# alenzhao/Mitty

Measured on NVIDIA B200. Metric: read pairs/sec (2x150, FASTQ-formatted, corrupted), higher is better.
Workload: dtype u8

## Files before the change

mitty_b200/csrc/mg_api.cu:

```cuda
#include <algorithm>
#include <cmath>
#include <cstdarg>
#include <cstdio>
#include <cstring>
#include <ctime>
#include <cstdlib>
#include <condition_variable>
#include <deque>
#include <map>
#include <memory>
#include <mutex>
#include <string>
#include <thread>
#include <vector>

#include "../../include/mitty_b200.h"
#include "mg_internal.h"

namespace {

struct DevBuf {
  void *p = nullptr;
  size_t cap = 0;
  ~DevBuf() { if (p) cudaFree(p); }
// ... 43 lines not shown
  uint32_t *d_eblk = nullptr;
  int n_blk = 0; int64_t hap_words = 0, hap_len = 0;
  std::vector<MgSegOut> segs;
  std::vector<int64_t> seg_start1;
  mg_ctx *owner = nullptr;
  ~Copy();
};

struct Batch {
  std::unique_ptr<Region> R;
  std::unique_ptr<Copy> C;
};

const int BLK_SHIFT = 8;

}

struct mg_ctx {
  int device = 0;
  cudaStream_t stream = nullptr;
  bool own_stream = false;
  std::string err;
  DevBuf m_tlen, m_bq, m_phred, m_alias[2], m_tlen_alias;
  bool has_tlen_alias = false;
  int n_tlen = 0, n_mates = 0, n_cycles = 0, n_bq = 0, rlen = 0;
  std::vector<uint32_t> h_alias[2]; int a_kshift[2] = {0, 0}, a_code9[2] = {0, 0}, a_rows[2] = {0, 0};
  std::vector<std::pair<void *, size_t>> pool;
  size_t pool_bytes = 0;
  std::map<void *, size_t> block_size;
  std::map<int64_t, std::unique_ptr<Region>> regions;
  std::map<int64_t, std::unique_ptr<Copy>> copies;
  std::map<int64_t, std::unique_ptr<Batch>> batches;
  int64_t next_id = 1;
  DevBuf s_raw, s_exc, s_ts, s_u, s_fo, s_tsorted, s_partial, s_state, s_out[2][2], s_str, s_plan, s_sample[3];
  DevBuf c_in[2], c_out[2], c_nl[2], c_cnt, c_sz[2], c_off[2], c_tmp, c_draw[4];
  DevBuf b_units, b_arr;
  HostBuf h_stage;
  cudaEvent_t ev0 = nullptr, ev1 = nullptr, ev2 = nullptr;
  cudaStream_t copy_stream = nullptr;
  cudaEvent_t ev_d2h[2] = {nullptr, nullptr};
  int ob = 0;
  int last_ob = 0; int64_t last_bytes = 0;
  double plan_ms = 0;
  double emit_ms = 0; int64_t emit_launches = 0, emit_bytes = 0, total_launches = 0;
  struct DrainJob {
    mg_sink *sink; int producer; int64_t unit; int ob; int64_t bytes;
    std::shared_ptr<std::vector<int64_t>> units, base;
  };
  std::thread drain_thread;
  std::mutex dmu; std::condition_variable dcv;
  std::deque<DrainJob> djobs;
  int dbusy[2] = {0, 0};
  bool dstop = false, dfailed = false;
  std::string derr;
  cudaEvent_t ev_drain[2] = {nullptr, nullptr};
  double d_wait_slot_ms = 0, d_wait_copy_ms = 0, d_idle_ms = 0; int64_t d_bytes = 0;
};

namespace {

int fail(mg_ctx *c, int code, const char *fmt, ...) {
  char buf[512];
  va_list ap; va_start(ap, fmt); vsnprintf(buf, sizeof buf, fmt, ap); va_end(ap);
  if (c) c->err = buf;
  return code;
}

// ... 629 lines not shown
  MgUnitParams P; const Copy *C;
  int rc = fill_unit_params(ctx, d, P, &C, false);
  if (rc) return rc;
  if (!d->qname_prefix || !d->qname_mid) return fail(ctx, MG_EINVAL, "qname_prefix / qname_mid missing");
  if (d->corrupt && d->mode != MG_MODE_PHILOX) return fail(ctx, MG_EINVAL, "fused corruption draws from Philox: use mg_corrupt_fastq for deterministic mode");
  if (d->corrupt && ctx->rlen > ctx->n_cycles) return fail(ctx, MG_EINDEX, "read length %d exceeds the model's %d cycles", ctx->rlen, ctx->n_cycles);
  if (d->corrupt && ctx->n_mates < 2) return fail(ctx, MG_EINVAL, "paired corruption needs a 2-mate model");
  const size_t n = (size_t)d->n_candidates;
  const int pl = (int)strlen(d->qname_prefix), ml = (int)strlen(d->qname_mid);
  const int L = ctx->rlen;

  if (pl > MG_QN_MAX || ml > MG_QN_MAX) return fail(ctx, MG_EVALUE, "sample / chromosome name too long for the qname buffers (%d)", MG_QN_MAX);
  mg_qn_const(P.qn, reinterpret_cast<const uint8_t *>(d->qname_prefix), pl, reinterpret_cast<const uint8_t *>(d->qname_mid), ml, L);
  P.qn_len = pl + ml;
  {
    static const bool lsu = getenv("MG_COPYOUT_LSU") != nullptr;
    P.bulk = lsu ? 0 : 1;
  }
  P.corrupt = d->corrupt;
  P.cor.kshift = ctx->a_kshift[0]; P.cor.code9 = ctx->a_code9[0];
  P.cor.alias = ctx->m_alias[0].as<uint32_t>();
  P.cor.n_cycles = ctx->n_cycles; P.cor.n_mates = ctx->n_mates;
  P.cor.k0 = d->corrupt_seed; P.cor.k1 = d->unit_seed ^ 0x636f7231u;
  P.L_nd = mg_ndigits32((uint32_t)L);

  P.n_tiles = (int)((n + MG_PLAN_TILE - 1) / MG_PLAN_TILE);
  int stage = 32 * (2 * L + 5 + 96);
  if (stage > 48 * 1024) stage = 48 * 1024;
  P.stage_cap = stage & ~15;
  int smem = 0;
  const int grid = mg_unit_grid(L, d->corrupt ? 1 + P.cor.code9 : 0, P.stage_cap, &smem);
  if (grid <= 0) return fail(ctx, MG_EVALUE, "the emit kernel's staging area (%d bytes for reads of %d bases) exceeds the shared memory of this device", smem, L);

  const size_t state_bytes = 48 + 16 * (size_t)std::max(P.n_tiles, 1);
  CU(ctx->s_state.need(state_bytes));
  uint8_t *sb = ctx->s_state.as<uint8_t>();
  P.totals = reinterpret_cast<unsigned long long *>(sb);
  P.tile_counter = reinterpret_cast<uint32_t *>(sb + 32);
  P.descA = reinterpret_cast<unsigned long long *>(sb + 48);
  P.descB = P.descA + std::max(P.n_tiles, 1);
  CU(ctx->s_plan.need(sizeof(MgPlan) * std::max<size_t>(n, 1)));
  P.plan = ctx->s_plan.as<MgPlan>();

  size_t est = n * (size_t)(2 * L + 5 + pl + ml + 12 + 2 * 36) / 6 * 5 + 4096;
  const bool want_out = (out1 != nullptr) || (out2 != nullptr);
  unsigned long long tot[4] = {0, 0, 0, 0};
  CU(cudaMemsetAsync(sb, 0, state_bytes, ctx->stream));
  CU(cudaEventRecord(ctx->ev2, ctx->stream));
  mg_launch_plan(P, ctx->stream);
  CU(cudaGetLastError());
  {
    std::unique_lock<std::mutex> lk(ctx->dmu);
    while (ctx->dbusy[ctx->ob] > 0 && !ctx->dfailed) ctx->dcv.wait(lk);
    if (ctx->dfailed) return fail(ctx, MG_EVALUE, "output sink: %s", ctx->derr.c_str());
  }
  for (int attempt = 0; attempt < 2; attempt++) {
    DevBuf *ob = ctx->s_out[ctx->ob];
    if (ob[0].cap < est || ob[1].cap < est) CU(cudaStreamSynchronize(ctx->copy_stream));
    CU(ob[0].need(est)); CU(ob[1].need(est));
    P.out[0] = ob[0].as<uint8_t>(); P.out[1] = ob[1].as<uint8_t>();
    P.cap = std::min(ob[0].cap, ob[1].cap);
    CU(cudaStreamWaitEvent(ctx->stream, ctx->ev_d2h[ctx->ob], 0));
    CU(cudaEventRecord(ctx->ev0, ctx->stream));
    mg_launch_unit(P, grid, smem, ctx->stream);
    CU(cudaEventRecord(ctx->ev1, ctx->stream));
    CU(cudaGetLastError());
    CU(cudaMemcpyAsync(tot, P.totals, sizeof tot, cudaMemcpyDeviceToHost, ctx->stream));
    CU(cudaStreamSynchronize(ctx->stream));
    if (P.n_tiles) {
      float ms = 0, ms_plan = 0;
      cudaEventElapsedTime(&ms, ctx->ev0, ctx->ev1);
      if (attempt == 0) { cudaEventElapsedTime(&ms_plan, ctx->ev2, ctx->ev0); ctx->plan_ms += ms_plan; ctx->total_launches++; }
      ctx->emit_ms += ms; ctx->emit_launches++; ctx->total_launches++;
      ctx->emit_bytes += 2 * (int64_t)tot[2];
    }
    if (!tot[3]) break;
    if (attempt == 1) return fail(ctx, MG_ECUDA, "internal: output overflow after regrow");
    est = (size_t)tot[2] + 4096;
    CU(cudaMemsetAsync(P.totals + 3, 0, 8, ctx->stream));
  }
  ctx->last_ob = ctx->ob; ctx->last_bytes = (int64_t)tot[2];
  if (n_bytes) *n_bytes = (int64_t)tot[2];
  if (n_templates) *n_templates = (int64_t)tot[1];
  if (n_te_kept) *n_te_kept = (int64_t)tot[0];
  if (!want_out) ctx->ob ^= 1;
  if (want_out) {
    if ((int64_t)tot[2] > cap) return fail(ctx, MG_ECAP, "output needs %lld bytes per file, caller gave %lld", (long long)tot[2], (long long)cap);
    if (out1 && tot[2]) CU(cudaMemcpyAsync(out1, P.out[0], (size_t)tot[2], cudaMemcpyDeviceToHost, ctx->copy_stream));
    if (out2 && tot[2]) CU(cudaMemcpyAsync(out2, P.out[1], (size_t)tot[2], cudaMemcpyDeviceToHost, ctx->copy_stream));
    CU(cudaEventRecord(ctx->ev_d2h[ctx->ob], ctx->copy_stream));
    ctx->ob ^= 1;
    if (wait_copies) CU(cudaStreamSynchronize(ctx->copy_stream));
  }
  return MG_OK;
}

int mg_unit_generate(mg_ctx *ctx, const mg_unit_desc *d, uint8_t *out1, uint8_t *out2, int64_t cap, int64_t *n_bytes,
                     int64_t *n_templates, int64_t *n_te_kept) {
  return unit_generate(ctx, d, out1, out2, cap, n_bytes, n_templates, n_te_kept, true);
}

int mg_unit_generate_async(mg_ctx *ctx, const mg_unit_desc *d, uint8_t *out1, uint8_t *out2, int64_t cap, int64_t *n_bytes,
                           int64_t *n_templates, int64_t *n_te_kept) {
  return unit_generate(ctx, d, out1, out2, cap, n_bytes, n_templates, n_te_kept, false);
}
// ... 488 lines not shown
```

mitty_b200/csrc/mg_core.cuh:

```cuda
#pragma once
#include <stdint.h>

#if defined(__CUDACC__)
#define MG_HD __host__ __device__ __forceinline__
#else
#define MG_HD inline
#endif
#if defined(__CUDACC__)
#define MG_NI static __host__ __device__ __noinline__ __attribute__((unused))
#else
#define MG_NI static __attribute__((noinline, unused))
#endif
#if defined(__CUDA_ARCH__)
#define MG_UNROLL _Pragma("unroll")
#define MG_NOUNROLL _Pragma("unroll 1")
#else
#define MG_UNROLL
#define MG_NOUNROLL
#endif


struct alignas(16) MgNode {
  uint32_t key;
  int32_t pr;
// ... 338 lines not shown
  MgTok A, B;
  mg_tok_num(v, pre, npre, A, B);
  w.append(A); w.append(B);
}

template <class SP>
MG_HD void mg_put_small(MgStream<SP> &w, uint32_t v, uint32_t pre, uint32_t npre) {
  if (v >= 10000u) { mg_put_num(w, v, pre, npre); return; }
  const uint32_t d = mg_dec4(v), x = d ^ 0x30303030u;
  uint32_t lz;
#if defined(__CUDA_ARCH__)
  lz = (x & 0x00FFFFFFu) ? ((uint32_t)__ffs((int)x) - 1u) >> 3 : 3u;
#else
  lz = (x & 0x00FFFFFFu) ? ((uint32_t)__builtin_ctz(x)) >> 3 : 3u;
#endif
  const uint32_t dig = d >> (8u * lz), ps = 8u * npre;
  MgTok t;
  t.lo = pre | (dig << ps); t.hi = mg_funnel_l(dig, 0u, ps); t.n = npre + 4u - lz;
  w.append(t);
}

MG_HD MgTok mg_tok(uint32_t lo, uint32_t hi, uint32_t n) { MgTok t; t.lo = lo; t.hi = hi; t.n = n; return t; }

template <class W>
MG_HD void mg_put_u32(W &w, uint32_t v) {
  uint64_t acc = 0;
  int n = 0;
  do { uint32_t q = v / 10u; acc = (acc << 4) | (v - q * 10u); v = q; n++; } while (v);
  for (; n; n--) { w.put((uint8_t)('0' + ((uint32_t)acc & 15u))); acc >>= 4; }
}


template <class NP, class BP>
MG_NI int mg_find_node(NP nodes, BP blk, int blk_shift, int n_blk, int n_nodes, uint32_t x) {
  uint32_t b = x >> blk_shift;
  if ((int)b >= n_blk) b = (uint32_t)(n_blk - 1);
  int lo = (int)blk[b];
  int hi = ((int)b + 1 < n_blk) ? (int)blk[b + 1] : n_nodes - 1;
  while (lo < hi) {
    int mid = (lo + hi + 1) >> 1;
    if (nodes[mid].key <= x) lo = mid; else hi = mid - 1;
  }
  return lo;
}

template <class NP>
MG_HD int mg_last_node(NP nodes, int n0, int n_nodes, uint32_t x, int L) {
  const uint32_t last = x + (uint32_t)L - 1u;
  int n1 = n0;
  while (n1 + 1 < n_nodes && nodes[n1 + 1].key <= last) n1++;
  return n1;
}

MG_HD int32_t mg_read_pos(const MgNode &f, bool single, uint32_t x) {
  if (f.op == 'I') return single ? f.pr - 1 : f.pr;
  const int64_t ps0 = (int64_t)f.key - (f.op == 'D' ? 1 : 0);
  return (int32_t)((int64_t)x - ps0 + (int64_t)f.pr);
}

MG_HD int32_t mg_cigar_len(const MgNode &n, uint32_t x, int L) {
  if (n.op == 'D') return n.oplen;
  int64_t a = (int64_t)x - (int64_t)n.key; if (a < 0) a = 0;
  int64_t b = (int64_t)x + L - (int64_t)n.key; if ((int64_t)n.oplen < b) b = n.oplen;
  return (int32_t)(b - a);
}

template <class W>
MG_HD void mg_put_i32(W &w, int32_t v) {
  if (v < 0) { w.put('-'); mg_put_u32(w, (uint32_t)(-(int64_t)v)); } else mg_put_u32(w, (uint32_t)v);
}

MG_HD int mg_nchars_i32(int32_t v) {
  const bool neg = v < 0;
  return (neg ? 1 : 0) + mg_ndigits32(neg ? (uint32_t)(-(int64_t)v) : (uint32_t)v);
}

template <class NP>
MG_NI uint32_t mg_read_fields_len(NP nodes, int n0, int n1, uint32_t x, int L, int L_nd) {
  const MgNode f = nodes[n0];
  const bool single = (n0 == n1);
  uint32_t n = 2u + 1u + (uint32_t)mg_nchars_i32(mg_read_pos(f, single, x)) + 1u + (uint32_t)L_nd + 1u + 1u;
  if (single && f.op == '=') return n + (uint32_t)L_nd + 1u;
  if (single && f.op == 'I')
    return n + 1u + (uint32_t)mg_nchars_i32((int32_t)((int64_t)x - (int64_t)f.key)) + 1u + (uint32_t)L_nd + 1u + (uint32_t)mg_nchars_i32(f.oplen);
  uint32_t nv = 0;
  for (int k = n0; k <= n1; k++) {
    const MgNode nd = nodes[k];
    n += (uint32_t)mg_nchars_i32(mg_cigar_len(nd, x, L)) + 1u;
    if (nd.op != '=') {
      n += (nv ? 1u : 0u) + (nd.op == 'X' ? 1u : nd.op == 'I' ? (uint32_t)mg_nchars_i32(nd.oplen) : (uint32_t)mg_nchars_i32(-nd.oplen));
      nv++;
    }
  }
  return n;
}

template <class W, class NP>
MG_HD void mg_fmt_read(W &w, NP nodes, int n0, int n1, uint32_t x, int L, int strand) {
  const MgNode f = nodes[n0];
  const bool single = (n0 == n1);
  w.put('|'); w.put((uint8_t)('0' + strand));
  w.put('|'); mg_put_i32(w, mg_read_pos(f, single, x));
  w.put('|'); mg_put_u32(w, (uint32_t)L);
  w.put('|');
  if (single && f.op == '=') {
    mg_put_u32(w, (uint32_t)L); w.put('='); w.put('|');
    return;
  }
  if (single && f.op == 'I') {
    w.put('>'); mg_put_i32(w, (int32_t)((int64_t)x - (int64_t)f.key)); w.put(':'); mg_put_u32(w, (uint32_t)L); w.put('I');
  } else {
    for (int k = n0; k <= n1; k++) {
      const MgNode n = nodes[k];
      mg_put_i32(w, mg_cigar_len(n, x, L)); w.put((uint8_t)n.op);
    }
  }
  w.put('|');
  bool first = true;
  for (int k = n0; k <= n1; k++) {
    const MgNode n = nodes[k];
    if (n.op == '=') continue;
    if (!first) w.put(',');
    first = false;
    if (n.op == 'X') w.put('0');
    else mg_put_i32(w, n.op == 'I' ? n.oplen : -n.oplen);
  }
}
// ... 146 lines not shown

template <class EP>
MG_HD int mg_exc_first(EP exc, int n_exc, uint32_t x) {
  int lo = 0, hi = n_exc;
  while (lo < hi) {
    int mid = (lo + hi) >> 1;
    if ((uint64_t)exc[mid].start + exc[mid].len <= (uint64_t)x) lo = mid + 1; else hi = mid;
  }
  return lo;
}

struct MgExcView {
  const MgExc *p; const uint32_t *blk; int shift, n_blk;
  MG_HD const MgExc &operator[](int k) const { return p[k]; }
};

MG_HD int mg_exc_first(MgExcView exc, int n_exc, uint32_t x) {
  int lo = 0, hi = n_exc;
  if (exc.blk) {
    uint32_t b = x >> exc.shift;
    if ((int)b > exc.n_blk - 1) b = (uint32_t)(exc.n_blk - 1);
    lo = (int)exc.blk[b]; hi = (int)exc.blk[b + 1];
    if (hi > n_exc) hi = n_exc;
    if (lo > hi) lo = hi;
  }
  while (lo < hi) {
    int mid = (lo + hi) >> 1;
    if ((uint64_t)exc.p[mid].start + exc.p[mid].len <= (uint64_t)x) lo = mid + 1; else hi = mid;
  }
  return lo;
}

template <class EP>
MG_NI int mg_count_N(EP exc, int n_exc, uint32_t x, int L, bool &touch) {
  int cnt = 0;
  touch = false;
  for (int k = mg_exc_first(exc, n_exc, x); k < n_exc; k++) {
    MgExc e = exc[k];
    if ((uint64_t)e.start >= (uint64_t)x + L) break;
    touch = true;
    if (e.byte != 'N') continue;
    uint64_t a = e.start > x ? e.start : x;
    uint64_t b = (uint64_t)e.start + e.len < (uint64_t)x + L ? (uint64_t)e.start + e.len : (uint64_t)x + L;
    cnt += (int)(b - a);
  }
  return cnt;
}

template <class HP>
MG_HD uint8_t mg_exc_byte(const MgExc &e, HP hap, uint64_t i) {
  if (e.byte != MG_EXC_CASE) return (uint8_t)e.byte;
  return (uint8_t)("acgt"[(hap[i >> 4] >> (2 * (i & 15))) & 3u]);
}

template <class HP>
struct MgCodeCursor {
  HP hap; uint64_t wi; uint32_t wv;
  MG_HD explicit MgCodeCursor(HP h) : hap(h), wi(~0ull), wv(0u) {}
  MG_HD uint32_t at(uint64_t i) {
    if ((i >> 4) != wi) { wi = i >> 4; wv = hap[wi]; }
    return (wv >> (2u * ((uint32_t)i & 15u))) & 3u;
  }
};

#define MG_CASE_WORDS 6
struct MgCaseMask {
  uint32_t m[MG_CASE_WORDS];
  MG_HD void clear() { MG_UNROLL for (int w = 0; w < MG_CASE_WORDS; w++) m[w] = 0u; }
  MG_HD void set(uint32_t lo, uint32_t hi) {
    MG_UNROLL
    for (int w = 0; w < MG_CASE_WORDS; w++) {
      const uint32_t l = lo > 32u * w ? lo - 32u * w : 0u, h = hi < 32u * w + 32u ? (hi > 32u * w ? hi - 32u * w : 0u) : 32u;
      if (l < h) m[w] |= (h - l == 32u ? 0xFFFFFFFFu : ((1u << (h - l)) - 1u) << l);
    }
  }
  MG_HD uint32_t next4() {
    const uint32_t b = m[0] & 15u;
    MG_UNROLL
    for (int w = 0; w + 1 < MG_CASE_WORDS; w++) m[w] = mg_funnel_r(m[w], m[w + 1], 4u);
// ... 348 lines not shown
```

mitty_b200/csrc/mg_internal.h:

```cpp
#pragma once
#include <cuda_runtime.h>
#include <stdint.h>
#include "mg_core.cuh"

#define MG_PLAN_TILE 256
#define MG_CTA 128
#define MG_TLEN_K 1024
#define MG_QN_MAX 192
#define MG_HAP_PAD 8

enum { MG_MODE_PHILOX = 0, MG_MODE_DET = 1, MG_MODE_EXPLICIT = 2 };

struct alignas(16) MgPlan {
  uint32_t xa, xb;
  int32_t n0a, n0b;
  uint32_t dn;
  uint32_t fo_sz;
  uint64_t off;
};

#define MG_BATCH_MAXC 2048
struct MgBatchUnit {
  MgTok pre[4], mid[4];
  int n_pre, n_mid;
  uint32_t qn_len;
  uint32_t seed;
  uint32_t x0, hap_len;
  uint32_t n_cand, plan_off;
  int64_t draw_off;
  int64_t p_min;
};

struct MgUnitParams {
  const uint32_t *hap;
  uint32_t hap_len;
  int64_t p_min;
  const MgNode *nodes; int n_nodes;
  const uint32_t *blk; int blk_shift; int n_blk;
  const MgExc *exc; int n_exc;
  const uint32_t *eblk;
  const double *cum_tlen; int n_tlen; int rlen;
  const uint32_t *tlen_alias;
  int mode; uint32_t n_cand;
  const int64_t *ts_in;
  const double *u_tlen;
  const int64_t *tl_in;
  const int8_t *fo_in;
  const uint32_t *ts_sorted;
  uint32_t key_tlen0, key_tlen1, key_perm0, key_perm1, perm_bits;
  MgQnConst qn;
  int qn_len;
  int bulk;
  uint8_t *out[2]; uint64_t cap;
  MgPlan *plan;
  int corrupt; MgCorruptCtx cor;
  int L_nd;
  unsigned long long *descA, *descB; uint32_t *tile_counter;
  unsigned long long *totals;
  int n_tiles; int stage_cap;
  const MgBatchUnit *bunits; int n_bunits;
  const long long *kept_base, *byte_base;
  long long *unit_kept, *unit_bytes, *unit_te;
  double inv_log1mp;
};

struct MgUnitKeys { uint32_t gap0, gap1, tlen0, tlen1, perm0, perm1, perm_bits; };
__host__ __device__ inline MgUnitKeys mg_unit_keys(uint32_t seed, uint32_t n_cand) {
  MgUnitKeys k;
  k.gap0 = seed; k.gap1 = 0x67617031u;
  k.tlen0 = seed; k.tlen1 = 0x746c6531u;
  k.perm0 = seed ^ 0x7368756bu; k.perm1 = seed * 0x9E3779B1u + 0x66656973u;
  k.perm_bits = mg_perm_bits(n_cand);
  return k;
}

struct MgSampleParams {
  MgUnitParams u;
  int64_t *ts_out; int64_t *te_out; int8_t *fo_out;
};

struct MgCorruptParams {
  const uint8_t *in[2]; uint8_t *out[2];
  const int64_t *nl[2];
  const int64_t *out_off[2];
  int64_t n_rec; int n_files;
  int64_t first;
  const double *cum_bq; int n_cycles, n_bq; const double *phred;
  int mode;
  MgCorruptCtx cor;
  const double *bq_rnd, *call_rnd; const uint8_t *base_rnd; const int64_t *draw_off;
// ... 15 lines not shown
  int32_t ends_in_d;
  uint32_t node0, n_nodes;
  uint32_t pad;
};
struct MgWalkSummary {
  unsigned long long err;
  long long n_nodes, hap_len;
  int32_t ends_in_d, bad;
};

struct MgWalkParams {
  const int64_t *pos, *oplen, *alt_off; const uint8_t *op;
  int n_var;
  const MgSeg *segs; int n_seg; MgSegOut *seg_out;
  uint32_t *nxt, *jump[2]; uint8_t *mark; int32_t *pred;
  int64_t *packed, *scanned, *scan_tmp;
  MgNode *nodes; uint32_t *node_alt;
  MgWalkSummary *sum;
};

int mg_launch_walk(const MgWalkParams &W, cudaStream_t st);
void mg_launch_exc_count(const MgNode *nodes, const uint32_t *node_alt, const MgWalkSummary *sum, int max_nodes,
                         const uint8_t *alt_pool, const MgExc *rexc, int n_rexc, int64_t *cnt, cudaStream_t st);
void mg_launch_exc_write(const MgNode *nodes, const uint32_t *node_alt, const MgWalkSummary *sum, int max_nodes,
                         const uint8_t *alt_pool, const MgExc *rexc, int n_rexc, int64_t *off, MgExc *out, cudaStream_t st);
void mg_launch_hap_build(const uint32_t *ref, const uint8_t *alt_pool, const MgNode *nodes, const uint32_t *node_alt,
                         int n_nodes, const uint32_t *blk, int blk_shift, int n_blk, uint32_t hap_len, uint32_t *hap, int64_t hap_words,
                         cudaStream_t st);
void mg_launch_blk_table(const MgNode *nodes, int n_nodes, uint32_t *blk, int n_blk, int blk_shift, cudaStream_t st);
void mg_launch_eblk_table(const MgExc *exc, int n_exc, uint32_t *eblk, int n_entries, int blk_shift, cudaStream_t st);
void mg_launch_gap_scan(uint32_t n, double p, uint32_t k0, uint32_t k1, uint32_t *ts_sorted, unsigned long long *partial,
                        cudaStream_t st);
int mg_unit_grid(int L, int corrupt, int stage_cap, int *smem_bytes);
void mg_launch_plan(const MgUnitParams &P, cudaStream_t st);
void mg_launch_unit(const MgUnitParams &P, int grid, int smem_bytes, cudaStream_t st);
void mg_launch_batch_plan(const MgUnitParams &P, cudaStream_t st);
int mg_batch_grid(int L, int corrupt, int stage_cap, int *smem_bytes);
void mg_launch_batch_emit(const MgUnitParams &P, int grid, int smem_bytes, cudaStream_t st);
void mg_launch_sample(const MgSampleParams &P, cudaStream_t st);
void mg_launch_scan_i64(const int64_t *in, int64_t *out, int64_t n, int64_t *tmp, cudaStream_t st);
int64_t mg_scan_tmp_elems(int64_t n);
void mg_launch_nl_count(const uint8_t *buf, int64_t len, int64_t *cnt, cudaStream_t st);
void mg_launch_nl_write(const uint8_t *buf, int64_t len, const int64_t *off, int64_t *nl, cudaStream_t st);
int64_t mg_nl_chunks(int64_t len);
void mg_launch_corrupt_sizes(const MgCorruptParams &P, int64_t *sz0, int64_t *sz1, cudaStream_t st);
void mg_launch_corrupt(const MgCorruptParams &P, cudaStream_t st);
void mg_launch_corrupt_staged(const MgCorruptParams &P, bool bulk, cudaStream_t st);
int mg_corrupt_stage_cap(void);
```

mitty_b200/csrc/mg_kernels.cu:

```cuda
#include <algorithm>
#include <cstdlib>
#include "mg_internal.h"

#define FULL 0xffffffffu


__device__ __forceinline__ uint32_t warp_incl_scan_u32(uint32_t v, int lane) {
#pragma unroll
  for (int d = 1; d < 32; d <<= 1) {
    uint32_t n = __shfl_up_sync(FULL, v, d);
    if (lane >= d) v += n;
  }
  return v;
}

__device__ __forceinline__ unsigned long long warp_sum_u64(unsigned long long v) {
#pragma unroll
  for (int d = 16; d >= 1; d >>= 1) v += __shfl_xor_sync(FULL, v, d);
  return v;
}

__device__ __forceinline__ unsigned long long ld_vol64(const unsigned long long *p) {
  return *(const volatile unsigned long long *)p;
}
__device__ __forceinline__ void st_vol64(unsigned long long *p, unsigned long long v) {
  *(volatile unsigned long long *)p = v;
}


__global__ void __launch_bounds__(256) k_pack_ref(const uint8_t *__restrict__ raw, int64_t len, uint32_t *__restrict__ packed,
                                                  uint32_t *exc_cnt, int64_t *exc_start, uint8_t *exc_byte,
                                                  int64_t *exc_end, uint32_t exc_cap) {
  int64_t w = (int64_t)blockIdx.x * blockDim.x + threadIdx.x;
  int64_t base = w * 16;
  if (base >= len) return;
  uint8_t c[18];
  c[0] = base > 0 ? raw[base - 1] : 0;
  if (base + 16 <= len) {
    uint4 v = *reinterpret_cast<const uint4 *>(raw + base);
    uint32_t q[4] = {v.x, v.y, v.z, v.w};
#pragma unroll
    for (int i = 0; i < 16; i++) c[1 + i] = (uint8_t)(q[i >> 2] >> (8 * (i & 3)));
  } else {
#pragma unroll
    for (int i = 0; i < 16; i++) c[1 + i] = (base + i < len) ? raw[base + i] : (uint8_t)'A';
  }
  c[17] = (base + 16 < len) ? raw[base + 16] : 0;
  uint32_t word = 0;
#pragma unroll
  for (int i = 0; i < 16; i++) {
    int64_t pos = base + i;
    if (pos >= len) break;
    uint32_t code = mg_base_code(c[1 + i]);
    if (code > 3) {
      const uint32_t lc = mg_base_code((uint8_t)(c[1 + i] ^ 0x20));
      const bool soft = c[1 + i] >= 'a' && lc <= 3;
      bool is_start, is_end;
      if (soft) {
        const bool prev_soft = pos > 0 && c[i] >= 'a' && mg_base_code((uint8_t)(c[i] ^ 0x20)) <= 3;
        const bool next_soft = pos < len - 1 && c[2 + i] >= 'a' && mg_base_code((uint8_t)(c[2 + i] ^ 0x20)) <= 3;
// ... 467 lines not shown
    }
    c.fo = r.v[2] & 1u;
  } else {
    c.ts_rel = P.ts_in[j] - P.p_min;
    tl = (P.mode == MG_MODE_DET) ? (int64_t)mg_lower_bound_f64(P.cum_tlen, P.n_tlen, P.u_tlen[j]) : P.tl_in[j];
  }
  if (tl < P.rlen) tl = P.rlen;
  c.te_rel = c.ts_rel + tl;
  c.k1 = (c.te_rel < (int64_t)P.hap_len) && (c.ts_rel >= 0);
  return c;
}

__global__ void __launch_bounds__(256) k_sample(MgSampleParams S) {
  __shared__ uint32_t s_tlen[MG_TLEN_K];
  if (S.u.mode == MG_MODE_PHILOX && S.u.tlen_alias)
    for (int i = threadIdx.x; i < MG_TLEN_K; i += blockDim.x) s_tlen[i] = S.u.tlen_alias[i];
  __syncthreads();
  for (uint32_t j = blockIdx.x * blockDim.x + threadIdx.x; j < S.u.n_cand; j += gridDim.x * blockDim.x) {
    Cand c = sample_candidate(S.u, s_tlen, j);
    S.ts_out[j] = c.ts_rel + S.u.p_min;
    S.te_out[j] = c.k1 ? c.te_rel + S.u.p_min : -1;
    S.fo_out[j] = (int8_t)c.fo;
  }
}

void mg_launch_sample(const MgSampleParams &P, cudaStream_t st) {
  if (P.u.n_cand == 0) return;
  int grid = (int)((P.u.n_cand + 255) / 256);
  if (grid > 148 * 8) grid = 148 * 8;
  k_sample<<<grid, 256, 0, st>>>(P);
}


struct Agg { unsigned long long c1, c2, by; };

#define DESC_FLAG(x) ((uint32_t)((x) >> 62))
#define DESC_MASK62 ((1ull << 62) - 1ull)

#define LOOKBACK_WIN 128
__device__ Agg tile_lookback(const MgUnitParams &P, int tile, int lane) {
  constexpr int Q = LOOKBACK_WIN / 32;
  Agg ex = {0, 0, 0};
  int idx = tile - 1;
  while (true) {
    unsigned long long a[Q], b[Q];
#pragma unroll
    for (int q = 0; q < Q; q++) {
      const int t = idx - 32 * q - lane;
      a[q] = 2ull << 62; b[q] = 2ull << 62;
      if (t >= 0) { a[q] = ld_vol64(P.descA + t); b[q] = ld_vol64(P.descB + t); }
    }
#pragma unroll
    for (int q = 0; q < Q; q++) {
      const int t = idx - 32 * q - lane;
      while (t >= 0 && (DESC_FLAG(a[q]) == 0 || DESC_FLAG(a[q]) != DESC_FLAG(b[q]))) {
        a[q] = ld_vol64(P.descA + t); b[q] = ld_vol64(P.descB + t);
      }
    }
    __syncwarp();
    int stop = LOOKBACK_WIN;
#pragma unroll
    for (int q = Q - 1; q >= 0; q--) {
      const uint32_t pm = __ballot_sync(FULL, DESC_FLAG(a[q]) == 2);
      if (pm) stop = 32 * q + __ffs(pm) - 1;
    }
    unsigned long long c1 = 0, c2 = 0, by = 0;
#pragma unroll
    for (int q = 0; q < Q; q++) {
      if (32 * q + lane <= stop) {
        c1 += (a[q] >> 31) & 0x7FFFFFFFull; c2 += a[q] & 0x7FFFFFFFull; by += b[q] & DESC_MASK62;
      }
    }
    ex.c1 += warp_sum_u64(c1); ex.c2 += warp_sum_u64(c2); ex.by += warp_sum_u64(by);
    if (stop < LOOKBACK_WIN) break;
    idx -= LOOKBACK_WIN;
  }
  return ex;
}

#define PLAN_THREADS 256

__global__ void __launch_bounds__(PLAN_THREADS, 6) k_unit_plan(const __grid_constant__ MgUnitParams P) {
  __shared__ uint32_t s_tlen[MG_TLEN_K];
  __shared__ uint4 s_hold[2][PLAN_THREADS];
  __shared__ uint2 s_hold2[2][PLAN_THREADS], s_ex[PLAN_THREADS];
  __shared__ uint32_t s_wc[2][PLAN_THREADS / 32], s_ws[2][PLAN_THREADS / 32];
  __shared__ unsigned long long s_base[2][3];
  __shared__ uint32_t s_tile[2];
  const int t = threadIdx.x, lane = t & 31, wid = t >> 5;
  const int L = P.rlen;
  if (P.mode == MG_MODE_PHILOX && P.tlen_alias) {
#pragma unroll 1
    for (int i = t; i < MG_TLEN_K; i += PLAN_THREADS) s_tlen[i] = P.tlen_alias[i];
  }
  if (t == 0) s_tile[0] = atomicAdd(P.tile_counter, 1u);
  __syncthreads();
  int tile = (int)s_tile[0], prev = -1;
  uint32_t prev_c1 = 0, prev_c2 = 0, prev_sz = 0;
#pragma unroll 1
  for (int k = 0;; k++) {
    const int cur = k & 1;
    const bool live = tile < P.n_tiles;
    if (t == 0 && live) s_tile[cur ^ 1] = atomicAdd(P.tile_counter, 1u);
    const uint32_t j = (uint32_t)tile * PLAN_THREADS + t;
    bool k1 = false, k2 = false, ta = false, tb = false;
    uint32_t xa = 0, xb = 0, fo = 0, sz = 0;
    int n0a = 0, n1a = 0, n0b = 0, n1b = 0;
    if (live && j < P.n_cand) {
      Cand c = sample_candidate(P, s_tlen, j);
      k1 = c.k1; fo = c.fo;
      if (k1) {
        xa = (uint32_t)c.ts_rel; xb = (uint32_t)(c.te_rel - L);
        k2 = true;
        if (P.n_exc) {
          const MgExcView ev = {P.exc, P.eblk, P.blk_shift, P.n_blk};
          const int na = mg_count_N(ev, P.n_exc, xa, L, ta), nb = mg_count_N(ev, P.n_exc, xb, L, tb);
          k2 = na <= 2 && nb <= 2;
        }
        if (k2) {
          n0a = mg_find_node(P.nodes, P.blk, P.blk_shift, P.n_blk, P.n_nodes, xa);
          n1a = mg_last_node(P.nodes, n0a, P.n_nodes, xa, L);
          n0b = mg_find_node(P.nodes, P.blk, P.blk_shift, P.n_blk, P.n_nodes, xb);
          n1b = mg_last_node(P.nodes, n0b, P.n_nodes, xb, L);
          sz = (uint32_t)P.qn_len + mg_read_fields_len(P.nodes, n0a, n1a, xa, L, P.L_nd) +
               mg_read_fields_len(P.nodes, n0b, n1b, xb, L, P.L_nd) + 2u * (uint32_t)L + 5u;
        }
      }
    }
    s_hold[cur][t] = make_uint4(xa, xb, (uint32_t)n0a, (uint32_t)n0b);
    s_hold2[cur][t] = make_uint2((uint32_t)(n1a - n0a) | ((uint32_t)(n1b - n0b) << 16),
                                 (fo << 31) | ((ta ? 1u : 0u) << 30) | ((tb ? 1u : 0u) << 29) | sz);
    const uint32_t cpk = (k1 ? 1u : 0u) | (k2 ? 0x10000u : 0u);
    const uint32_t ic = warp_incl_scan_u32(cpk, lane), is = warp_incl_scan_u32(sz, lane);
    if (lane == 31) { s_wc[cur][wid] = ic; s_ws[cur][wid] = is; }
    if (wid == 0 && prev >= 0) {
      Agg ex = {0, 0, 0};
      if (prev > 0) ex = tile_lookback(P, prev, lane);
      if (lane == 0) {
        const unsigned long long i1 = ex.c1 + prev_c1, i2 = ex.c2 + prev_c2, ib = ex.by + prev_sz;
        if (prev > 0) {
          st_vol64(P.descA + prev, (2ull << 62) | (i1 << 31) | i2);
          st_vol64(P.descB + prev, (2ull << 62) | ib);
        }
        s_base[cur ^ 1][0] = ex.c1; s_base[cur ^ 1][1] = ex.c2; s_base[cur ^ 1][2] = ex.by;
        if (prev == P.n_tiles - 1) { P.totals[0] = i1; P.totals[1] = i2; P.totals[2] = ib + mg_digit_sum(i2); }
      }
    }
    __syncthreads();
    if (prev >= 0) {
      const uint2 h1 = s_hold2[cur ^ 1][t];
      if (h1.y & 0x1FFFFFFFu) {
        const uint4 h0 = s_hold[cur ^ 1][t];
        const uint2 ex = s_ex[t];
        const unsigned long long base1 = s_base[cur ^ 1][0], base2 = s_base[cur ^ 1][1];
        const unsigned long long rank = base2 + (ex.x >> 16);
        const unsigned long long off = s_base[cur ^ 1][2] + ex.y + mg_digit_sum(rank);
        const uint32_t my_fo = (P.mode == MG_MODE_PHILOX) ? h1.y >> 31 : (uint32_t)(P.fo_in[base1 + (ex.x & 0xFFFFu)] & 1);
        MgPlan pl;
        pl.xa = h0.x; pl.xb = h0.y; pl.n0a = (int32_t)h0.z; pl.n0b = (int32_t)h0.w;
        pl.dn = h1.x;
        pl.fo_sz = (my_fo << 31) | ((h1.y & 0x7FFFFFFFu) + (uint32_t)mg_ndigits32((uint32_t)(rank + 1)));
        pl.off = off;
        P.plan[rank] = pl;
      }
    }
    if (!live) break;
    uint32_t oc = 0, os = 0, tc = 0, ts_ = 0;
#pragma unroll
    for (int w = 0; w < PLAN_THREADS / 32; w++) {
      if (w < wid) { oc += s_wc[cur][w]; os += s_ws[cur][w]; }
      tc += s_wc[cur][w]; ts_ += s_ws[cur][w];
    }
    const uint32_t ec = oc + ic - cpk, es = os + is - sz;
    prev_c1 = tc & 0xFFFFu; prev_c2 = tc >> 16; prev_sz = ts_;
    if (t == 0) {
      const unsigned long long fl = tile == 0 ? 2ull << 62 : 1ull << 62;
      st_vol64(P.descA + tile, fl | ((unsigned long long)prev_c1 << 31) | prev_c2);
      st_vol64(P.descB + tile, fl | prev_sz);
    }
    s_ex[t] = make_uint2(ec, es);
    prev = tile;
    tile = (int)s_tile[cur ^ 1];
  }
}

void mg_launch_plan(const MgUnitParams &P, cudaStream_t st) {
  if (P.n_tiles == 0) return;
  static const int resident = [] {
    int dev = 0, sms = 0, per_sm = 0;
    cudaGetDevice(&dev);
    cudaDeviceGetAttribute(&sms, cudaDevAttrMultiProcessorCount, dev);
    cudaOccupancyMaxActiveBlocksPerMultiprocessor(&per_sm, k_unit_plan, PLAN_THREADS, 0);
    return std::max(1, sms * per_sm);
  }();
  k_unit_plan<<<std::min(P.n_tiles, resident), PLAN_THREADS, 0, st>>>(P);
}

__global__ void __launch_bounds__(PLAN_THREADS) k_batch_plan(const __grid_constant__ MgUnitParams P) {
  __shared__ uint32_t s_ts[MG_BATCH_MAXC];
  __shared__ uint32_t s_tlen[MG_TLEN_K];
  __shared__ unsigned long long s_w64[PLAN_THREADS / 32];
  __shared__ uint32_t s_wc[PLAN_THREADS / 32], s_ws[PLAN_THREADS / 32];
  __shared__ unsigned long long s_carry[3];
  const int t = threadIdx.x, lane = t & 31, wid = t >> 5;
  const int L = P.rlen;
  const MgBatchUnit U = P.bunits[blockIdx.x];
  const uint32_t n = U.n_cand;
  const MgUnitKeys K = mg_unit_keys(U.seed, n);
  if (P.mode == MG_MODE_PHILOX) {
    if (P.tlen_alias) for (int i = t; i < MG_TLEN_K; i += PLAN_THREADS) s_tlen[i] = P.tlen_alias[i];
    uint32_t g[8];
    unsigned long long sum = 0;
    const uint32_t i0 = (uint32_t)t * 8u;
    if (i0 < n) { gaps8(i0, n, P.inv_log1mp, K.gap0, K.gap1, g); for (int q = 0; q < 8; q++) sum += g[q]; }
    else { for (int q = 0; q < 8; q++) g[q] = 0; }
    unsigned long long x = sum;
#pragma unroll
    for (int d = 1; d < 32; d <<= 1) { unsigned long long y = __shfl_up_sync(FULL, x, d); if (lane >= d) x += y; }
    if (lane == 31) s_w64[wid] = x;
    __syncthreads();
    unsigned long long run = x - sum;
    for (int w = 0; w < wid; w++) run += s_w64[w];
    for (int q = 0; q < 8; q++) {
      run += g[q];
      if (i0 + q < n) { const unsigned long long v = run + 1; s_ts[i0 + q] = v > 0xFFFFFFFFull ? 0xFFFFFFFFu : (uint32_t)v; }
    }
  }
  if (t == 0) { s_carry[0] = 0; s_carry[1] = 0; s_carry[2] = 0; }
  __syncthreads();
  for (uint32_t c0 = 0; c0 < n; c0 += PLAN_THREADS) {
// ... 720 lines not shown
```

Baseline: 1.419 billion.

## Replace single-pass decoupled-lookback plan kernel with count/scan/place three-kernel pipeline

Replaces the persistent plan kernel, which used dynamic tile counters and decoupled lookback, with three launches. A count kernel stores per-candidate hold records to global memory and writes per-tile aggregates. A single-block kernel scans those aggregates, and a place kernel computes ranks and offsets and writes the plan. This removes the serial lookback spin-waiting and the volatile descriptor traffic, and inlines the helper functions in the hot path. In exchange it adds two extra launches, a 24-byte-per-candidate global round trip, and a single-block scan step. It also drops shared-memory staging of the tlen alias table.

```diff
diff --git a/mitty_b200/csrc/mg_api.cu b/mitty_b200/csrc/mg_api.cu
--- a/mitty_b200/csrc/mg_api.cu
+++ b/mitty_b200/csrc/mg_api.cu
@@ -99,7 +99,7 @@
   std::map<int64_t, std::unique_ptr<Copy>> copies;
   std::map<int64_t, std::unique_ptr<Batch>> batches;
   int64_t next_id = 1;
-  DevBuf s_raw, s_exc, s_ts, s_u, s_fo, s_tsorted, s_partial, s_state, s_out[2][2], s_str, s_plan, s_sample[3];
+  DevBuf s_raw, s_exc, s_ts, s_u, s_fo, s_tsorted, s_partial, s_state, s_out[2][2], s_str, s_plan, s_hold, s_sample[3];
   DevBuf c_in[2], c_out[2], c_nl[2], c_cnt, c_sz[2], c_off[2], c_tmp, c_draw[4];
   DevBuf b_units, b_arr;
   HostBuf h_stage;
@@ -795,22 +795,22 @@
   const int grid = mg_unit_grid(L, d->corrupt ? 1 + P.cor.code9 : 0, P.stage_cap, &smem);
   if (grid <= 0) return fail(ctx, MG_EVALUE, "the emit kernel's staging area (%d bytes for reads of %d bases) exceeds the shared memory of this device", smem, L);
 
-  const size_t state_bytes = 48 + 16 * (size_t)std::max(P.n_tiles, 1);
-  CU(ctx->s_state.need(state_bytes));
+  CU(ctx->s_state.need(32 + 16 * (size_t)std::max(P.n_tiles, 1)));
   uint8_t *sb = ctx->s_state.as<uint8_t>();
   P.totals = reinterpret_cast<unsigned long long *>(sb);
-  P.tile_counter = reinterpret_cast<uint32_t *>(sb + 32);
-  P.descA = reinterpret_cast<unsigned long long *>(sb + 48);
-  P.descB = P.descA + std::max(P.n_tiles, 1);
+  P.tile_agg = reinterpret_cast<ulonglong2 *>(sb + 32);
   CU(ctx->s_plan.need(sizeof(MgPlan) * std::max<size_t>(n, 1)));
   P.plan = ctx->s_plan.as<MgPlan>();
+  CU(ctx->s_hold.need(MG_HOLD_BYTES * std::max<size_t>(n, 1)));
+  P.hold0 = ctx->s_hold.as<uint4>();
+  P.hold1 = reinterpret_cast<uint2 *>(P.hold0 + std::max<size_t>(n, 1));
 
   size_t est = n * (size_t)(2 * L + 5 + pl + ml + 12 + 2 * 36) / 6 * 5 + 4096;
   const bool want_out = (out1 != nullptr) || (out2 != nullptr);
   unsigned long long tot[4] = {0, 0, 0, 0};
-  CU(cudaMemsetAsync(sb, 0, state_bytes, ctx->stream));
+  CU(cudaMemsetAsync(P.totals, 0, 32, ctx->stream));
   CU(cudaEventRecord(ctx->ev2, ctx->stream));
-  mg_launch_plan(P, ctx->stream);
+  const int plan_launches = mg_launch_plan(P, ctx->stream);
   CU(cudaGetLastError());
   {
     std::unique_lock<std::mutex> lk(ctx->dmu);
@@ -833,7 +833,7 @@
     if (P.n_tiles) {
       float ms = 0, ms_plan = 0;
       cudaEventElapsedTime(&ms, ctx->ev0, ctx->ev1);
-      if (attempt == 0) { cudaEventElapsedTime(&ms_plan, ctx->ev2, ctx->ev0); ctx->plan_ms += ms_plan; ctx->total_launches++; }
+      if (attempt == 0) { cudaEventElapsedTime(&ms_plan, ctx->ev2, ctx->ev0); ctx->plan_ms += ms_plan; ctx->total_launches += plan_launches; }
       ctx->emit_ms += ms; ctx->emit_launches++; ctx->total_launches++;
       ctx->emit_bytes += 2 * (int64_t)tot[2];
     }
diff --git a/mitty_b200/csrc/mg_core.cuh b/mitty_b200/csrc/mg_core.cuh
--- a/mitty_b200/csrc/mg_core.cuh
+++ b/mitty_b200/csrc/mg_core.cuh
@@ -394,7 +394,7 @@
 
 
 template <class NP, class BP>
-MG_NI int mg_find_node(NP nodes, BP blk, int blk_shift, int n_blk, int n_nodes, uint32_t x) {
+MG_HD int mg_find_node_i(NP nodes, BP blk, int blk_shift, int n_blk, int n_nodes, uint32_t x) {
   uint32_t b = x >> blk_shift;
   if ((int)b >= n_blk) b = (uint32_t)(n_blk - 1);
   int lo = (int)blk[b];
@@ -405,6 +405,10 @@
   }
   return lo;
 }
+template <class NP, class BP>
+MG_NI int mg_find_node(NP nodes, BP blk, int blk_shift, int n_blk, int n_nodes, uint32_t x) {
+  return mg_find_node_i(nodes, blk, blk_shift, n_blk, n_nodes, x);
+}
 
 template <class NP>
 MG_HD int mg_last_node(NP nodes, int n0, int n_nodes, uint32_t x, int L) {
@@ -438,7 +442,7 @@
 }
 
 template <class NP>
-MG_NI uint32_t mg_read_fields_len(NP nodes, int n0, int n1, uint32_t x, int L, int L_nd) {
+MG_HD uint32_t mg_read_fields_len_i(NP nodes, int n0, int n1, uint32_t x, int L, int L_nd) {
   const MgNode f = nodes[n0];
   const bool single = (n0 == n1);
   uint32_t n = 2u + 1u + (uint32_t)mg_nchars_i32(mg_read_pos(f, single, x)) + 1u + (uint32_t)L_nd + 1u + 1u;
@@ -455,6 +459,10 @@
     }
   }
   return n;
+}
+template <class NP>
+MG_NI uint32_t mg_read_fields_len(NP nodes, int n0, int n1, uint32_t x, int L, int L_nd) {
+  return mg_read_fields_len_i(nodes, n0, n1, x, L, L_nd);
 }
 
 template <class W, class NP>
@@ -667,7 +675,7 @@
 }
 
 template <class EP>
-MG_NI int mg_count_N(EP exc, int n_exc, uint32_t x, int L, bool &touch) {
+MG_HD int mg_count_N_i(EP exc, int n_exc, uint32_t x, int L, bool &touch) {
   int cnt = 0;
   touch = false;
   for (int k = mg_exc_first(exc, n_exc, x); k < n_exc; k++) {
@@ -680,6 +688,10 @@
     cnt += (int)(b - a);
   }
   return cnt;
+}
+template <class EP>
+MG_NI int mg_count_N(EP exc, int n_exc, uint32_t x, int L, bool &touch) {
+  return mg_count_N_i(exc, n_exc, x, L, touch);
 }
 
 template <class HP>
diff --git a/mitty_b200/csrc/mg_internal.h b/mitty_b200/csrc/mg_internal.h
--- a/mitty_b200/csrc/mg_internal.h
+++ b/mitty_b200/csrc/mg_internal.h
@@ -4,6 +4,7 @@
 #include "mg_core.cuh"
 
 #define MG_PLAN_TILE 256
+#define MG_HOLD_BYTES 24
 #define MG_CTA 128
 #define MG_TLEN_K 1024
 #define MG_QN_MAX 192
@@ -55,7 +56,7 @@
   MgPlan *plan;
   int corrupt; MgCorruptCtx cor;
   int L_nd;
-  unsigned long long *descA, *descB; uint32_t *tile_counter;
+  uint4 *hold0; uint2 *hold1; ulonglong2 *tile_agg;
   unsigned long long *totals;
   int n_tiles; int stage_cap;
   const MgBatchUnit *bunits; int n_bunits;
@@ -137,7 +138,7 @@
 void mg_launch_gap_scan(uint32_t n, double p, uint32_t k0, uint32_t k1, uint32_t *ts_sorted, unsigned long long *partial,
                         cudaStream_t st);
 int mg_unit_grid(int L, int corrupt, int stage_cap, int *smem_bytes);
-void mg_launch_plan(const MgUnitParams &P, cudaStream_t st);
+int mg_launch_plan(const MgUnitParams &P, cudaStream_t st);
 void mg_launch_unit(const MgUnitParams &P, int grid, int smem_bytes, cudaStream_t st);
 void mg_launch_batch_plan(const MgUnitParams &P, cudaStream_t st);
 int mg_batch_grid(int L, int corrupt, int stage_cap, int *smem_bytes);
diff --git a/mitty_b200/csrc/mg_kernels.cu b/mitty_b200/csrc/mg_kernels.cu
--- a/mitty_b200/csrc/mg_kernels.cu
+++ b/mitty_b200/csrc/mg_kernels.cu
@@ -20,12 +20,6 @@
   return v;
 }
 
-__device__ __forceinline__ unsigned long long ld_vol64(const unsigned long long *p) {
-  return *(const volatile unsigned long long *)p;
-}
-__device__ __forceinline__ void st_vol64(unsigned long long *p, unsigned long long v) {
-  *(volatile unsigned long long *)p = v;
-}
 
 
 __global__ void __launch_bounds__(256) k_pack_ref(const uint8_t *__restrict__ raw, int64_t len, uint32_t *__restrict__ packed,
@@ -559,170 +553,143 @@
 }
 
 
-struct Agg { unsigned long long c1, c2, by; };
-
-#define DESC_FLAG(x) ((uint32_t)((x) >> 62))
-#define DESC_MASK62 ((1ull << 62) - 1ull)
-
-#define LOOKBACK_WIN 128
-__device__ Agg tile_lookback(const MgUnitParams &P, int tile, int lane) {
-  constexpr int Q = LOOKBACK_WIN / 32;
-  Agg ex = {0, 0, 0};
-  int idx = tile - 1;
-  while (true) {
-    unsigned long long a[Q], b[Q];
-#pragma unroll
-    for (int q = 0; q < Q; q++) {
-      const int t = idx - 32 * q - lane;
-      a[q] = 2ull << 62; b[q] = 2ull << 62;
-      if (t >= 0) { a[q] = ld_vol64(P.descA + t); b[q] = ld_vol64(P.descB + t); }
-    }
-#pragma unroll
-    for (int q = 0; q < Q; q++) {
-      const int t = idx - 32 * q - lane;
-      while (t >= 0 && (DESC_FLAG(a[q]) == 0 || DESC_FLAG(a[q]) != DESC_FLAG(b[q]))) {
-        a[q] = ld_vol64(P.descA + t); b[q] = ld_vol64(P.descB + t);
-      }
-    }
-    __syncwarp();
-    int stop = LOOKBACK_WIN;
-#pragma unroll
-    for (int q = Q - 1; q >= 0; q--) {
-      const uint32_t pm = __ballot_sync(FULL, DESC_FLAG(a[q]) == 2);
-      if (pm) stop = 32 * q + __ffs(pm) - 1;
-    }
-    unsigned long long c1 = 0, c2 = 0, by = 0;
-#pragma unroll
-    for (int q = 0; q < Q; q++) {
-      if (32 * q + lane <= stop) {
-        c1 += (a[q] >> 31) & 0x7FFFFFFFull; c2 += a[q] & 0x7FFFFFFFull; by += b[q] & DESC_MASK62;
-      }
-    }
-    ex.c1 += warp_sum_u64(c1); ex.c2 += warp_sum_u64(c2); ex.by += warp_sum_u64(by);
-    if (stop < LOOKBACK_WIN) break;
-    idx -= LOOKBACK_WIN;
-  }
-  return ex;
-}
-
-#define PLAN_THREADS 256
-
-__global__ void __launch_bounds__(PLAN_THREADS, 6) k_unit_plan(const __grid_constant__ MgUnitParams P) {
-  __shared__ uint32_t s_tlen[MG_TLEN_K];
-  __shared__ uint4 s_hold[2][PLAN_THREADS];
-  __shared__ uint2 s_hold2[2][PLAN_THREADS], s_ex[PLAN_THREADS];
-  __shared__ uint32_t s_wc[2][PLAN_THREADS / 32], s_ws[2][PLAN_THREADS / 32];
-  __shared__ unsigned long long s_base[2][3];
-  __shared__ uint32_t s_tile[2];
+
+__global__ void __launch_bounds__(MG_PLAN_TILE, 8) k_plan_count(const __grid_constant__ MgUnitParams P) {
+  __shared__ uint32_t s_c[MG_PLAN_TILE / 32], s_s[MG_PLAN_TILE / 32];
   const int t = threadIdx.x, lane = t & 31, wid = t >> 5;
   const int L = P.rlen;
-  if (P.mode == MG_MODE_PHILOX && P.tlen_alias) {
-#pragma unroll 1
-    for (int i = t; i < MG_TLEN_K; i += PLAN_THREADS) s_tlen[i] = P.tlen_alias[i];
-  }
-  if (t == 0) s_tile[0] = atomicAdd(P.tile_counter, 1u);
+  const uint32_t j = blockIdx.x * MG_PLAN_TILE + t;
+  bool k1 = false, k2 = false, ta = false, tb = false;
+  uint32_t xa = 0, xb = 0, fo = 0, sz = 0;
+  int n0a = 0, n1a = 0, n0b = 0, n1b = 0;
+  if (j < P.n_cand) {
+    Cand c = sample_candidate(P, P.tlen_alias, j);
+    k1 = c.k1; fo = c.fo;
+    if (k1) {
+      xa = (uint32_t)c.ts_rel; xb = (uint32_t)(c.te_rel - L);
+      k2 = true;
+      if (P.n_exc) {
+        const MgExcView ev = {P.exc, P.eblk, P.blk_shift, P.n_blk};
+        const int na = mg_count_N_i(ev, P.n_exc, xa, L, ta), nb = mg_count_N_i(ev, P.n_exc, xb, L, tb);
+        k2 = na <= 2 && nb <= 2;
+      }
+      if (k2) {
+        n0a = mg_find_node_i(P.nodes, P.blk, P.blk_shift, P.n_blk, P.n_nodes, xa);
+        n1a = mg_last_node(P.nodes, n0a, P.n_nodes, xa, L);
+        n0b = mg_find_node_i(P.nodes, P.blk, P.blk_shift, P.n_blk, P.n_nodes, xb);
+        n1b = mg_last_node(P.nodes, n0b, P.n_nodes, xb, L);
+        sz = (uint32_t)P.qn_len + mg_read_fields_len_i(P.nodes, n0a, n1a, xa, L, P.L_nd) +
+             mg_read_fields_len_i(P.nodes, n0b, n1b, xb, L, P.L_nd) + 2u * (uint32_t)L + 5u;
+      }
+    }
+    const uint32_t bit31 = P.mode == MG_MODE_PHILOX ? fo : (k1 ? 1u : 0u);
+    P.hold0[j] = make_uint4(xa, xb, (uint32_t)n0a, (uint32_t)n0b);
+    P.hold1[j] = make_uint2((uint32_t)(n1a - n0a) | ((uint32_t)(n1b - n0b) << 16),
+                            (bit31 << 31) | ((ta ? 1u : 0u) << 30) | ((tb ? 1u : 0u) << 29) | sz);
+  }
+  const uint32_t wc = __reduce_add_sync(FULL, (k1 ? 1u : 0u) | (k2 ? 0x10000u : 0u)), ws = __reduce_add_sync(FULL, sz);
+  if (lane == 0) { s_c[wid] = wc; s_s[wid] = ws; }
   __syncthreads();
-  int tile = (int)s_tile[0], prev = -1;
-  uint32_t prev_c1 = 0, prev_c2 = 0, prev_sz = 0;
-#pragma unroll 1
-  for (int k = 0;; k++) {
-    const int cur = k & 1;
-    const bool live = tile < P.n_tiles;
-    if (t == 0 && live) s_tile[cur ^ 1] = atomicAdd(P.tile_counter, 1u);
-    const uint32_t j = (uint32_t)tile * PLAN_THREADS + t;
-    bool k1 = false, k2 = false, ta = false, tb = false;
-    uint32_t xa = 0, xb = 0, fo = 0, sz = 0;
-    int n0a = 0, n1a = 0, n0b = 0, n1b = 0;
-    if (live && j < P.n_cand) {
-      Cand c = sample_candidate(P, s_tlen, j);
-      k1 = c.k1; fo = c.fo;
-      if (k1) {
-        xa = (uint32_t)c.ts_rel; xb = (uint32_t)(c.te_rel - L);
-        k2 = true;
-        if (P.n_exc) {
-          const MgExcView ev = {P.exc, P.eblk, P.blk_shift, P.n_blk};
-          const int na = mg_count_N(ev, P.n_exc, xa, L, ta), nb = mg_count_N(ev, P.n_exc, xb, L, tb);
-          k2 = na <= 2 && nb <= 2;
-        }
-        if (k2) {
-          n0a = mg_find_node(P.nodes, P.blk, P.blk_shift, P.n_blk, P.n_nodes, xa);
-          n1a = mg_last_node(P.nodes, n0a, P.n_nodes, xa, L);
-          n0b = mg_find_node(P.nodes, P.blk, P.blk_shift, P.n_blk, P.n_nodes, xb);
-          n1b = mg_last_node(P.nodes, n0b, P.n_nodes, xb, L);
-          sz = (uint32_t)P.qn_len + mg_read_fields_len(P.nodes, n0a, n1a, xa, L, P.L_nd) +
-               mg_read_fields_len(P.nodes, n0b, n1b, xb, L, P.L_nd) + 2u * (uint32_t)L + 5u;
-        }
-      }
-    }
-    s_hold[cur][t] = make_uint4(xa, xb, (uint32_t)n0a, (uint32_t)n0b);
-    s_hold2[cur][t] = make_uint2((uint32_t)(n1a - n0a) | ((uint32_t)(n1b - n0b) << 16),
-                                 (fo << 31) | ((ta ? 1u : 0u) << 30) | ((tb ? 1u : 0u) << 29) | sz);
-    const uint32_t cpk = (k1 ? 1u : 0u) | (k2 ? 0x10000u : 0u);
-    const uint32_t ic = warp_incl_scan_u32(cpk, lane), is = warp_incl_scan_u32(sz, lane);
-    if (lane == 31) { s_wc[cur][wid] = ic; s_ws[cur][wid] = is; }
-    if (wid == 0 && prev >= 0) {
-      Agg ex = {0, 0, 0};
-      if (prev > 0) ex = tile_lookback(P, prev, lane);
-      if (lane == 0) {
-        const unsigned long long i1 = ex.c1 + prev_c1, i2 = ex.c2 + prev_c2, ib = ex.by + prev_sz;
-        if (prev > 0) {
-          st_vol64(P.descA + prev, (2ull << 62) | (i1 << 31) | i2);
-          st_vol64(P.descB + prev, (2ull << 62) | ib);
-        }
-        s_base[cur ^ 1][0] = ex.c1; s_base[cur ^ 1][1] = ex.c2; s_base[cur ^ 1][2] = ex.by;
-        if (prev == P.n_tiles - 1) { P.totals[0] = i1; P.totals[1] = i2; P.totals[2] = ib + mg_digit_sum(i2); }
-      }
-    }
-    __syncthreads();
-    if (prev >= 0) {
-      const uint2 h1 = s_hold2[cur ^ 1][t];
-      if (h1.y & 0x1FFFFFFFu) {
-        const uint4 h0 = s_hold[cur ^ 1][t];
-        const uint2 ex = s_ex[t];
-        const unsigned long long base1 = s_base[cur ^ 1][0], base2 = s_base[cur ^ 1][1];
-        const unsigned long long rank = base2 + (ex.x >> 16);
-        const unsigned long long off = s_base[cur ^ 1][2] + ex.y + mg_digit_sum(rank);
-        const uint32_t my_fo = (P.mode == MG_MODE_PHILOX) ? h1.y >> 31 : (uint32_t)(P.fo_in[base1 + (ex.x & 0xFFFFu)] & 1);
-        MgPlan pl;
-        pl.xa = h0.x; pl.xb = h0.y; pl.n0a = (int32_t)h0.z; pl.n0b = (int32_t)h0.w;
-        pl.dn = h1.x;
-        pl.fo_sz = (my_fo << 31) | ((h1.y & 0x7FFFFFFFu) + (uint32_t)mg_ndigits32((uint32_t)(rank + 1)));
-        pl.off = off;
-        P.plan[rank] = pl;
-      }
-    }
-    if (!live) break;
-    uint32_t oc = 0, os = 0, tc = 0, ts_ = 0;
-#pragma unroll
-    for (int w = 0; w < PLAN_THREADS / 32; w++) {
-      if (w < wid) { oc += s_wc[cur][w]; os += s_ws[cur][w]; }
-      tc += s_wc[cur][w]; ts_ += s_ws[cur][w];
-    }
-    const uint32_t ec = oc + ic - cpk, es = os + is - sz;
-    prev_c1 = tc & 0xFFFFu; prev_c2 = tc >> 16; prev_sz = ts_;
-    if (t == 0) {
-      const unsigned long long fl = tile == 0 ? 2ull << 62 : 1ull << 62;
-      st_vol64(P.descA + tile, fl | ((unsigned long long)prev_c1 << 31) | prev_c2);
-      st_vol64(P.descB + tile, fl | prev_sz);
-    }
-    s_ex[t] = make_uint2(ec, es);
-    prev = tile;
-    tile = (int)s_tile[cur ^ 1];
-  }
-}
-
-void mg_launch_plan(const MgUnitParams &P, cudaStream_t st) {
-  if (P.n_tiles == 0) return;
-  static const int resident = [] {
-    int dev = 0, sms = 0, per_sm = 0;
-    cudaGetDevice(&dev);
-    cudaDeviceGetAttribute(&sms, cudaDevAttrMultiProcessorCount, dev);
-    cudaOccupancyMaxActiveBlocksPerMultiprocessor(&per_sm, k_unit_plan, PLAN_THREADS, 0);
-    return std::max(1, sms * per_sm);
-  }();
-  k_unit_plan<<<std::min(P.n_tiles, resident), PLAN_THREADS, 0, st>>>(P);
-}
-
+  if (t == 0) {
+    uint32_t tc = 0, tsz = 0;
+#pragma unroll
+    for (int w = 0; w < MG_PLAN_TILE / 32; w++) { tc += s_c[w]; tsz += s_s[w]; }
+    P.tile_agg[blockIdx.x] = make_ulonglong2(((unsigned long long)(tc & 0xFFFFu) << 32) | (tc >> 16), tsz);
+  }
+}
+
+#define PLAN_SCAN_THREADS 1024
+#define PLAN_SCAN_BATCH 8
+__global__ void __launch_bounds__(PLAN_SCAN_THREADS) k_plan_scan(const __grid_constant__ MgUnitParams P) {
+  __shared__ unsigned long long s_a[PLAN_SCAN_THREADS / 32], s_b[PLAN_SCAN_THREADS / 32];
+  const int t = threadIdx.x, lane = t & 31, wid = t >> 5;
+  const int per = (P.n_tiles + PLAN_SCAN_THREADS / 32 - 1) / (PLAN_SCAN_THREADS / 32);
+  const int i0 = min(wid * per, P.n_tiles), i1 = min(i0 + per, P.n_tiles);
+  unsigned long long sa = 0, sb = 0;
+  for (int g = i0; g < i1; g += 32 * PLAN_SCAN_BATCH) {
+    ulonglong2 v[PLAN_SCAN_BATCH];
+#pragma unroll
+    for (int q = 0; q < PLAN_SCAN_BATCH; q++) {
+      const int i = g + 32 * q + lane;
+      v[q] = i < i1 ? P.tile_agg[i] : make_ulonglong2(0ull, 0ull);
+    }
+#pragma unroll
+    for (int q = 0; q < PLAN_SCAN_BATCH; q++) { sa += v[q].x; sb += v[q].y; }
+  }
+  sa = warp_sum_u64(sa); sb = warp_sum_u64(sb);
+  if (lane == 0) { s_a[wid] = sa; s_b[wid] = sb; }
+  __syncthreads();
+  unsigned long long ra = 0, rb = 0, ta = 0, tb = 0;
+#pragma unroll
+  for (int w = 0; w < PLAN_SCAN_THREADS / 32; w++) {
+    if (w < wid) { ra += s_a[w]; rb += s_b[w]; }
+    ta += s_a[w]; tb += s_b[w];
+  }
+  if (t == 0) {
+    const unsigned long long kept = ta & 0xFFFFFFFFull;
+    P.totals[0] = ta >> 32; P.totals[1] = kept; P.totals[2] = tb + mg_digit_sum(kept);
+  }
+  for (int g = i0; g < i1; g += 32 * PLAN_SCAN_BATCH) {
+    ulonglong2 v[PLAN_SCAN_BATCH];
+#pragma unroll
+    for (int q = 0; q < PLAN_SCAN_BATCH; q++) {
+      const int i = g + 32 * q + lane;
+      v[q] = i < i1 ? P.tile_agg[i] : make_ulonglong2(0ull, 0ull);
+    }
+#pragma unroll
+    for (int q = 0; q < PLAN_SCAN_BATCH; q++) {
+      const int i = g + 32 * q + lane;
+      unsigned long long xa = v[q].x, xb = v[q].y;
+#pragma unroll
+      for (int d = 1; d < 32; d <<= 1) {
+        const unsigned long long ya = __shfl_up_sync(FULL, xa, d), yb = __shfl_up_sync(FULL, xb, d);
+        if (lane >= d) { xa += ya; xb += yb; }
+      }
+      if (i < i1) P.tile_agg[i] = make_ulonglong2(ra + xa - v[q].x, rb + xb - v[q].y);
+      ra += __shfl_sync(FULL, xa, 31); rb += __shfl_sync(FULL, xb, 31);
+    }
+  }
+}
+
+__global__ void __launch_bounds__(MG_PLAN_TILE, 8) k_plan_place(const __grid_constant__ MgUnitParams P) {
+  __shared__ uint32_t s_wc[MG_PLAN_TILE / 32], s_ws[MG_PLAN_TILE / 32];
+  const int t = threadIdx.x, lane = t & 31, wid = t >> 5;
+  const uint32_t j = blockIdx.x * MG_PLAN_TILE + t;
+  const uint2 h1 = j < P.n_cand ? P.hold1[j] : make_uint2(0u, 0u);
+  const uint32_t sz = h1.y & 0x1FFFFFFFu;
+  const uint32_t k1 = P.mode == MG_MODE_PHILOX ? 0u : h1.y >> 31;
+  const uint32_t cpk = k1 | (sz ? 0x10000u : 0u);
+  ulonglong2 base = make_ulonglong2(0ull, 0ull);
+  uint4 h0 = make_uint4(0u, 0u, 0u, 0u);
+  if (sz) { base = P.tile_agg[blockIdx.x]; h0 = P.hold0[j]; }
+  const uint32_t ic = warp_incl_scan_u32(cpk, lane), is = warp_incl_scan_u32(sz, lane);
+  if (lane == 31) { s_wc[wid] = ic; s_ws[wid] = is; }
+  __syncthreads();
+  if (!sz) return;
+  uint32_t ec = ic - cpk, es = is - sz;
+#pragma unroll
+  for (int w = 0; w < MG_PLAN_TILE / 32; w++)
+    if (w < wid) { ec += s_wc[w]; es += s_ws[w]; }
+  const unsigned long long rank = (base.x & 0xFFFFFFFFull) + (ec >> 16);
+  const unsigned long long off = base.y + es + mg_digit_sum(rank);
+  const uint32_t my_fo = (P.mode == MG_MODE_PHILOX) ? h1.y >> 31 : (uint32_t)(P.fo_in[(base.x >> 32) + (ec & 0xFFFFu)] & 1);
+  MgPlan pl;
+  pl.xa = h0.x; pl.xb = h0.y; pl.n0a = (int32_t)h0.z; pl.n0b = (int32_t)h0.w;
+  pl.dn = h1.x;
+  pl.fo_sz = (my_fo << 31) | ((h1.y & 0x7FFFFFFFu) + (uint32_t)mg_ndigits32((uint32_t)(rank + 1)));
+  pl.off = off;
+  P.plan[rank] = pl;
+}
+
+int mg_launch_plan(const MgUnitParams &P, cudaStream_t st) {
+  if (P.n_tiles == 0) return 0;
+  k_plan_count<<<P.n_tiles, MG_PLAN_TILE, 0, st>>>(P);
+  k_plan_scan<<<1, PLAN_SCAN_THREADS, 0, st>>>(P);
+  k_plan_place<<<P.n_tiles, MG_PLAN_TILE, 0, st>>>(P);
+  return 3;
+}
+
+#define PLAN_THREADS 256
 __global__ void __launch_bounds__(PLAN_THREADS) k_batch_plan(const __grid_constant__ MgUnitParams P) {
   __shared__ uint32_t s_ts[MG_BATCH_MAXC];
   __shared__ uint32_t s_tlen[MG_TLEN_K];
```

Result: faster. 1.456 billion, median of 6 (+2.7%).
